# daemon-219/ReID-GAN

Measured on AMD Instinct MI355X. Metric: train-step images/sec, 256×128 ReID batch, 1/2/4/8 MI355X, higher is better.
Workload: dtype f32; 1 GPU; FD-GAN G + D_id/D_pd fwd/bwd step (FDGANModel.optimize_parameters), batch 16 pairs = 32 crops of 256x128 + 18-ch pose map per GPU, stage 2, drop 0.2; crops_per_gpu=32, global_batch_crops=32, parallelism=dp1

## Files before the change

### include/reidgan_hip.h

```cpp
#ifndef REIDGAN_HIP_H
#define REIDGAN_HIP_H

#include <stddef.h>
#include <stdint.h>

#ifdef __cplusplus
extern "C" {
#endif

typedef struct ihipStream_t* rg_stream_t;

#define RG_OK 0
#define RG_ERR_INVALID (-1)
#define RG_ERR_LAUNCH (-2)
#define RG_ERR_WORKSPACE (-3)

#define RG_ACT_NONE 0
#define RG_ACT_RELU 1
#define RG_ACT_LEAKY 2
#define RG_ACT_TANH 3

const char* rg_last_error(void);
int rg_version(void);

// ... 7 lines not shown
int rg_conv2d_fwd(const float* x, const float* w, const float* w_krsc, float* y, int N, int C, int H, int W, int K,
                  int KH, int KW, int SH, int SW, int PH, int PW, int P, int Q, const float* scale, const float* shift,
                  const float* residual, int act, float slope, void* workspace, size_t workspace_bytes,
                  rg_stream_t stream);
size_t rg_conv2d_dgrad_workspace(int N, int C, int H, int W, int K, int KH, int KW, int SH, int SW);
int rg_conv2d_dgrad(const float* dy, const float* w, const float* w_krsc, float* dx, int N, int C, int H, int W, int K,
                    int KH, int KW, int SH, int SW, int PH, int PW, int P, int Q, const float* scale,
                    const float* shift, const float* residual, int act, float slope, const float* relu_mask,
                    float* rowsum, int rowsum_cols, void* workspace, size_t workspace_bytes, rg_stream_t stream);
int rg_conv2d_dgrad_rowsum_cols(int N, int C, int H, int W, int K, int KH, int KW, int SH, int SW, int PH, int PW, int P,
                                int Q);
int rg_weights_to_krsc(const float* w, float* w_krsc, int K, int C, int KH, int KW, rg_stream_t stream);
int rg_krsc_chunk(void);
int rg_weights_to_krsc_multi(const void* table, int count, int total_blocks, rg_stream_t stream);
int rg_conv_set_force(int tile, int splits);
int rg_conv_set_planes(int mask);
int rg_conv_tune_stats(int* out);
int rg_conv_set_pick(int kind, int index);
int rg_conv_pick_log(int* buf, int max_records);
int rg_conv_splitk_arrivals(void* counters, int count, rg_stream_t stream);
int rg_conv_splitk_inkernel_count(void);
size_t rg_conv2d_wgrad_workspace(int N, int C, int K, int KH, int KW, int P, int Q);
int rg_conv2d_wgrad(const float* x, const float* dy, float* dw, int N, int C, int H, int W, int K, int KH, int KW,
                    int SH, int SW, int PH, int PW, int P, int Q, void* workspace, size_t workspace_bytes,
                    rg_stream_t stream);

size_t rg_bn_workspace(int N, int C, int HW);
int rg_bn_stats(const float* x, float* mean, float* invstd, float* running_mean, float* running_var, int N, int C,
                int HW, float eps, float momentum, void* workspace, size_t workspace_bytes, rg_stream_t stream);
int rg_bn_apply_fwd(const float* x, const float* mean, const float* stat, const float* gamma, const float* beta,
// ... 243 lines not shown
```

### reid-gan_amd/csrc/conv_igemm.hip

```cpp
#include "conv_plan.h"

#include <stdio.h>
#include <string.h>
#include <atomic>
#include <map>
#include <mutex>
#include <vector>

namespace rg {
namespace conv {

const Switches& switches() {
    static const Switches s = {
        env_int("RG_CONV_TUNE", 1),     env_int("RG_CONV_TUNE_PLAN", 1), env_int("RG_CONV_TUNE_PATH", 1), env_int("RG_CONV_TUNE8", 1),
        env_int("RG_CONV_HALO", 1),     env_int("RG_HALO_WG", 512),
        env_int("RG_THIN_CONV", 1),     env_int("RG_THIN_PX4", 1),       env_int("RG_SMALLC_PX", 1),      env_int("RG_CONV_DMA", 1),
        env_int("RG_SPLITK_VEC", 1),    env_int("RG_DGRAD_STRIDED_SPLIT", 1),
        env_int("RG_WGRAD_WG", 1024),   env_int("RG_WGRAD_XCD", 1),      env_int("RG_WGRAD_RSC", 0),      env_int("RG_WGRAD_SHIFT", 1),
        env_int("RG_WGRAD_FOLD_FUSED", 1), getenv("RG_WGRAD_WG") != nullptr,
    };
    return s;
}

static bool fits_buffer(int64_t elems) { return elems > 0 && elems * 4 < (1ll << 31); }

int validate(const char* op, const ConvGeom& g) {
    const int N = g.N, C = g.C, H = g.H, W = g.W, K = g.K, KH = g.KH, KW = g.KW, SH = g.SH, SW = g.SW, PH = g.PH, PW = g.PW, P = g.P, Q = g.Q;
    RG_REQUIRE(N > 0 && C > 0 && H > 0 && W > 0 && K > 0 && KH > 0 && KW > 0, "%s: non-positive dimension", op);
    RG_REQUIRE(SH > 0 && SW > 0 && PH >= 0 && PW >= 0 && P > 0 && Q > 0, "%s: bad stride/pad/output size", op);
    RG_REQUIRE((P - 1) * SH - PH + KH - 1 >= 0 && (Q - 1) * SW - PW + KW - 1 >= 0, "%s: inconsistent geometry", op);
    RG_REQUIRE((int64_t)(P - 1) * SH - PH < H && (int64_t)(Q - 1) * SW - PW < W, "%s: output larger than input allows", op);
    RG_REQUIRE((int64_t)N * P * Q < (1ll << 31) && (int64_t)C * KH * KW < (1ll << 31) && (int64_t)N * H * W < (1ll << 31) &&
                   (int64_t)C * H * W < (1ll << 31) && (int64_t)K * P * Q < (1ll << 31) &&
                   (int64_t)K * KH * KW < (1ll << 31),
// ... 92 lines not shown
        }
    return n;
}
size_t plans_workspace(const Plan* pl, int n, int M, int64_t Ng) {
    size_t need = 0;
    for (int i = 0; i < n; ++i) {
        const size_t b = splitk_bytes(pl[i].splits, M, Ng);
        if (b > need) need = b;
    }
    return need;
}

static Plan plan_wgrad(int M, int Ng, int64_t Kg) {
    Plan pl;
    pl.tile = (M <= 32) ? 3 : ((M <= 64 || Ng <= 64) ? 2 : 0);
    pl.m_tiles = rg::cdiv(M, kTileBM[pl.tile]);
    pl.n_tiles = rg::cdiv(Ng, kTileBN[pl.tile]);
    const int64_t nk = rg::cdiv64(Kg, BK);
    const int64_t mn = (int64_t)pl.m_tiles * pl.n_tiles;
    int64_t want = rg::cdiv64(switches().wgrad_wg, mn);
    if (want > nk / 16) want = nk / 16;
    if (want < 1) want = 1;
    if (want > 512) want = 512;
    while (want > 1 && want * (int64_t)M * Ng * 4 >= (1ll << 31)) --want;
    if (switches().wgrad_xcd && want >= 8) {
        int64_t w8 = (want + 4) / 8 * 8;
        while (w8 > 8 && w8 * (int64_t)M * Ng * 4 >= (1ll << 31)) w8 -= 8;
        if (w8 * (int64_t)M * Ng * 4 < (1ll << 31) && w8 <= nk) {
            pl.ktiles_per_split = (int)rg::cdiv64(nk, w8);
            pl.splits = (int)w8;
            return pl;
        }
    }
    pl.ktiles_per_split = (int)rg::cdiv64(nk, want);
    pl.splits = (int)rg::cdiv64(nk, pl.ktiles_per_split);
    return pl;
}

int wgrad_plan_candidates(int M, int Ng, int64_t Kg, Plan* out, int max_out) {
    out[0] = plan_wgrad(M, Ng, Kg);
    int n = 1;
    if (!plan_tune_enabled() || switches().wgrad_wg_set) return n;
    if (2.0 * M * (double)Ng * (double)Kg < kPlanTuneMinFlop) return n;
    const int64_t nk = rg::cdiv64(Kg, BK);
    const int base = out[0].splits;
    const int alts[4] = {base / 2, base * 3 / 4, base * 3 / 2, base * 2};
    for (int i = 0; i < 4 && n < max_out; ++i) {
        int64_t sp = alts[i];
        if (sp >= 8) sp = (sp + 4) / 8 * 8;
        if (sp < 1) sp = 1;
        if (sp > 512) sp = 512;
        if (sp > 1 && nk / sp < 8) continue;
        if (sp * (int64_t)M * Ng * 4 >= (1ll << 31)) continue;
        Plan pl = out[0];
        pl.ktiles_per_split = (int)rg::cdiv64(nk, sp);
        pl.splits = sp >= 8 ? (int)sp : (int)rg::cdiv64(nk, pl.ktiles_per_split);
        if (pl.splits > nk) continue;
        bool dup = false;
        for (int j = 0; j < n; ++j) dup = dup || out[j].splits == pl.splits;
        if (!dup) out[n++] = pl;
    }
    return n;
}

struct Arrivals { unsigned* ptr; int count; };
static std::map<hipStream_t, Arrivals> g_arrivals;
static std::mutex g_arrivals_mu;
static std::atomic<int> g_inkernel_launches{0};
unsigned* splitk_arrivals(hipStream_t stream, int tiles) {
    Arrivals a = {nullptr, 0};
    {
        std::lock_guard<std::mutex> lock(g_arrivals_mu);
        auto it = g_arrivals.find(stream);
        if (it != g_arrivals.end()) a = it->second;
    }
    if (!a.ptr || tiles > a.count) return nullptr;
    hipStreamCaptureStatus cs = hipStreamCaptureStatusNone;
    if (hipStreamIsCapturing(stream, &cs) != hipSuccess || cs != hipStreamCaptureStatusNone) {
        (void)hipGetLastError();
// ... 119 lines not shown
    pick_record(key, ncand, c);
    return c;
}

}
}

using namespace rg::conv;

extern "C" int rg_conv_set_force(int tile, int splits) {
    g_force_tile = tile;
    g_force_splits = splits;
    return RG_OK;
}

extern "C" int rg_conv_set_planes(int mask) {
    const int old = planes_mask();
    planes_mask() = mask & 15;
    return old;
}

extern "C" int rg_conv_set_pick(int kind, int index) {
    const int slot = pick_slot(kind);
    if (slot < 0 || index < -1) {
        rg::set_error("rg_conv_set_pick: kind %d / index %d (kinds 1, 2, 4, 16, 32, 64, 128, 256; index >= -1)", kind, index);
        return RG_ERR_INVALID - 1;
    }
    std::lock_guard<std::mutex> lock(g_pick_mu);
    const int old = g_pick[slot].exchange(index);
    if ((old >= 0) != (index >= 0)) g_pick_pinned += index >= 0 ? 1 : -1;
// ... 32 lines not shown
```

### reid-gan_amd/csrc/conv_plan.h

```cpp
#pragma once
#include "rg_common.h"

#include <array>

namespace rg {
namespace conv {

constexpr int BK = 16;
constexpr int kTileBM[4] = {128, 64, 64, 32};
constexpr int kTileBN[4] = {128, 128, 64, 256};
constexpr int kMaxCand = 16;

struct ConvGeom {
    int N, C, H, W, K, KH, KW, SH, SW, PH, PW, P, Q;
};
inline double alg_bytes(const ConvGeom& g) {
    return 4.0 * ((double)g.N * g.C * g.H * g.W + (double)g.K * g.C * g.KH * g.KW + (double)g.N * g.K * g.P * g.Q);
}
int validate(const char* op, const ConvGeom& g);

struct Workspace {
    void* ptr;
    size_t bytes;
    bool holds(size_t need) const { return need <= bytes && (!need || ptr); }
};

template <typename... P>
inline bool aligned16(const P*... p) {
    return ((... | reinterpret_cast<uintptr_t>(p)) & 15) == 0;
}

struct Switches {
    int tune, tune_plan, tune_path, tune8;
    int halo, halo_wg;
    int thin, thin_px4, smallc_px, dma;
    int splitk_vec, strided_split;
    int wgrad_wg, wgrad_xcd, wgrad_rsc, wgrad_shift, fold_fused;
    bool wgrad_wg_set;
};
const Switches& switches();
inline bool path_tune_enabled() { return switches().tune && switches().tune_path; }

struct Plan {
    int tile, m_tiles, n_tiles, splits, ktiles_per_split;
};
inline size_t splitk_bytes(int splits, int M, int64_t Ng) { return splits > 1 ? (size_t)splits * M * (size_t)Ng * sizeof(float) : 0; }
inline size_t fit_splits(Plan& pl, int M, int64_t Ng, const Workspace& ws, size_t limit = ~(size_t)0) {
    const size_t need = splitk_bytes(pl.splits, M, Ng);
    if (need < limit && ws.holds(need)) return need;
    pl.splits = 1;
    pl.ktiles_per_split = 1 << 30;
    return 0;
}
Plan plan_gemm(int M, int64_t Ng, int64_t Kg, bool allow_split);
int plan_candidates(int M, int64_t Ng, int64_t Kg, Plan* out, int max_out);
int wgrad_plan_candidates(int M, int Ng, int64_t Kg, Plan* out, int max_out);
size_t plans_workspace(const Plan* pl, int n, int M, int64_t Ng);

typedef std::array<int, 16> TuneKey;
inline TuneKey tune_key(int kind, const ConvGeom& g, int f12, int f13, int f14, int f15) {
    return TuneKey{kind, g.N, g.C, g.H, g.W, g.K, g.KH, g.KW, g.SH, g.SW, g.PH, g.PW, f12, f13, f14, f15};
}

int choose_impl(int family_bit, const TuneKey& key, hipStream_t stream, int ncand, void (*run)(void*, int), void* ctx);
template <typename Run>
inline int choose_impl(int family_bit, const TuneKey& key, hipStream_t stream, int ncand, Run run) {
    return choose_impl(family_bit, key, stream, ncand, [](void* ctx, int c) { (*static_cast<Run*>(ctx))(c); }, &run);
}
template <typename Run>
inline int choose_status(const TuneKey& key, hipStream_t stream, int ncand, Run run) {
    if (ncand <= 1) return run(0);
    int st = RG_OK;
// ... 12 lines not shown
```

### reid-gan_amd/csrc/conv_planes.h

```cpp
#pragma once
#include "conv_planes_core.h"

#ifdef RG_PLANES_FWD
template <int BM, int BN, int WM, int WN, int BMODE, bool AVEC>
__global__ __launch_bounds__(64 * WM * WN) void conv_fwd_pl_kernel(const ConvP p) {
    using T = Tile<BM, BN, WM, WN>;
    constexpr int NTH = 64 * WM * WN;
    static_assert(BN >= 64, "the gather loader needs a wave-uniform k");
    using LA = PlTile<PL_R, BM>;
    using LB = PlTile<BMODE == 2 ? PL_T : PL_R, BN>;
    constexpr int TILEB = LA::BYTES + LB::BYTES;
    __shared__ __attribute__((aligned(16))) unsigned char lds[2 * TILEB];
    const unsigned lds0 = (unsigned)(size_t)((lds_u8_t*)lds);

    const int tid = threadIdx.x, lane = tid & 63, wid = tid >> 6;
    const int wm = wid / WN, wn = wid % WN;
    const int tile = xcd_remap(blockIdx.x, gridDim.x);
    const int mt = tile % p.m_tiles, nt = tile / p.m_tiles;
    const int m0 = mt * BM, n0 = nt * BN;
    const int split = blockIdx.y;
    const int HW = p.H * p.W;
    const int RS = p.KH * p.KW;
    const rsrc_t rw = make_rsrc(p.w, p.w_bytes), rx = make_rsrc(p.x, p.x_bytes);

// ... 359 lines not shown
        ob[j] = OOB;
        if (nn < cl.Ngc) {
            const int im = fdiv(nn, cl.d_hw);
            const int rem = nn - im * cl.Hc * cl.Wc;
            const int hc = fdiv(rem, cl.d_w);
            const int wc = rem - hc * cl.Wc;
            const int h = ah + p.SH * hc, w = aw + p.SW * wc;
            ob[j] = (unsigned)((((int64_t)im * p.C + mrow0) * HW + h * p.W + w) * 4);
        }
    }
    store_tile_epilogue_any<T>(p, acc, ob, (unsigned)HW * 4u, mrow0, (cl.poff + nt) * WN + wn);
}
#endif

#ifdef RG_PLANES_WGRAD
template <int BM, int BN, int WM, int WN, bool VEC, bool VECA>
__global__ __launch_bounds__(64 * WM * WN) void conv_wgrad_pl_kernel(const ConvP p) {
    using T = Tile<BM, BN, WM, WN>;
    constexpr int NTH = 64 * WM * WN;
    static_assert(BN >= 64, "the gather loader needs a wave-uniform pixel chunk");
    using LA = PlTile<PL_R, BM>;
    using LB = PlTile<PL_R, BN>;
    constexpr int TILEB = LA::BYTES + LB::BYTES;
    __shared__ __attribute__((aligned(16))) unsigned char lds[2 * TILEB];
    const unsigned lds0 = (unsigned)(size_t)((lds_u8_t*)lds);

    const int tid = threadIdx.x, lane = tid & 63, wid = tid >> 6;
    const int wm = wid / WN, wn = wid % WN;
    int tile_id, split;
    if ((gridDim.z & 7) == 0) {
        const unsigned lin = blockIdx.z * gridDim.x + blockIdx.x;
        const unsigned xcd = lin & 7, idx = lin >> 3;
        split = (int)(xcd + 8 * (idx / gridDim.x));
        tile_id = (int)(idx % gridDim.x);
    } else {
        split = blockIdx.z;
        tile_id = xcd_remap(blockIdx.x, gridDim.x);
    }
    const int mt = tile_id % p.m_tiles, nt = tile_id / p.m_tiles;
    const int m0 = mt * BM, n0 = nt * BN;
    const rsrc_t rdy = make_rsrc(p.w, p.w_bytes), rx = make_rsrc(p.x, p.x_bytes);
    const int PQ = p.P * p.Q, HW = p.H * p.W, RS = p.KH * p.KW;
    const bool rsc = p.a_vec4 != 0;
    const bool nopad = p.PH == 0 && p.PW == 0 && (p.P - 1) * p.SH + p.KH <= p.H && (p.Q - 1) * p.SW + p.KW <= p.W;

    constexpr int AVN = (BM * 4 + NTH - 1) / NTH;
    constexpr bool AFULL = BM * 4 >= NTH;
    constexpr int EA = BM * BK / NTH;
    static_assert(VECA || EA >= 2, "scalar chunk of at least one pair");
    PlStager<VECA ? AVN : 1, VECA ? 2 : EA / 2> sa;
    const int vrow = tid >> 2, vkq = (tid & 3) * 4;
    const bool aact = AFULL || vrow < BM;
    unsigned avoff[VECA ? AVN : 1];
// ... 116 lines not shown
                const int h0 = pp * p.SH - p.PH, w0 = qq * p.SW - p.PW;
                const int xb = img * p.C * HW + h0 * p.W + w0;
                const bool ok = gvalid && cvalid && (nopad || ((unsigned)(h0 + cr) < (unsigned)p.H && (unsigned)(w0 + cs) < (unsigned)p.W));
                rb[e] = bload(rx, ok ? (unsigned)(xb + coff) * 4u : OOB);
                if (++qq == p.Q) {
                    qq = 0;
                    if (++pp == p.P) { pp = 0; ++img; }
                }
            }
        }
    };

    constexpr int SA = decltype(sa)::STEPS, S = SA + decltype(sb)::STEPS;
    const unsigned fa = lds0 + LA::frag_base(lane, wm * T::WTM), fb = lds0 + LA::BYTES + LB::frag_base(lane, wn * T::WTN);
    const int nk_total = (p.Kg + BK - 1) / BK;
    const int kt_begin = split * p.ktiles_per_split;
    int kt_end = kt_begin + p.ktiles_per_split;
    if (kt_end > nk_total) kt_end = nk_total;
    pl_mainloop<T, LA, LB, S>(fa, fb, kt_begin, kt_end, acc, load_tile, [&](unsigned wbuf, int s) {
        if (s < SA) {
            if constexpr (AFULL || !VECA) sa.step(s, ra, wbuf, LA::PIECE);
            else sa.step(s, ra, wbuf, LA::PIECE, aact);
        } else {
            sb.step(s - SA, rb, wbuf, LB::PIECE);
        }
    });

    const int l32 = lane & 31, kh = lane >> 5;
    const rsrc_t ro = make_rsrc(p.y, p.y_bytes);
    const int mrow0 = m0 + wm * T::WTM + 4 * kh;
    const unsigned rstride = (unsigned)p.Ng * 4u;
#pragma unroll
    for (int j = 0; j < T::TN; ++j) {
        const int nn = n0 + wn * T::WTN + j * 32 + l32;
        const unsigned ob = nn < p.Ng ? (unsigned)((((int64_t)split * p.M + mrow0) * p.Ng + nn) * 4) : OOB;
#pragma unroll
        for (int i = 0; i < T::TM; ++i)
#pragma unroll
            for (int r = 0; r < 16; ++r) {
                const int mo = i * 32 + (r & 3) + 8 * (r >> 2);
                bstore(ro, (mrow0 + mo < p.M) ? ob + (unsigned)mo * rstride : OOB, acc[i][j][r]);
            }
    }
}
#endif
```

### reid-gan_amd/csrc/conv_planes_core.h

```cpp
#pragma once

enum { PL_R = 0, PL_T = 1 };

typedef int int2r __attribute__((ext_vector_type(2)));
typedef short short4r __attribute__((ext_vector_type(4)));
typedef __attribute__((address_space(3))) short4r lds_short4_t;
typedef __attribute__((address_space(3))) int4r lds_int4_t;
typedef __attribute__((address_space(3))) int2r lds_int2_t;
typedef __attribute__((address_space(3))) int lds_int_t;
typedef __attribute__((address_space(3))) unsigned char lds_u8_t;
template <bool B> struct BoolTag { static constexpr bool value = B; };

constexpr int pl_tpitch(int rows) {
    const int p = rows * 2, b = p / 256 * 256;
    return b + 64 >= p ? b + 64 : (b + 192 >= p ? b + 192 : b + 320);
}

template <int KIND, int ROWS>
struct PlTile {
    static constexpr int HALF = ROWS * 16 + 64;
    static constexpr int PITCH = pl_tpitch(ROWS);
    static constexpr int PIECE = KIND == PL_R ? 2 * HALF : 16 * PITCH;
    static constexpr int BYTES = 3 * PIECE;
    static constexpr int BLK = KIND == PL_R ? 512 : 64;
// ... 292 lines not shown
    __syncthreads();
    pl_kloop(kt_begin, kt_end, load_tile, [&](auto cur_tag, auto stage_tag) {
        constexpr int RD = decltype(cur_tag)::value ? TILEB : 0, WR = TILEB - RD;
        constexpr bool STAGE = decltype(stage_tag)::value;
        mma_pl16<T::TM, T::TN>([&](int i, int pc) { return LA::frag(fa[i & 1] + RD + pc * LA::PIECE + (i >> 1) * 2 * LA::BLK); },
                               [&](int j, int pc) { return LB::frag(fb[j & 1] + RD + pc * LB::PIECE + (j >> 1) * 2 * LB::BLK); }, acc,
                               [&](int slot) {
                                   if (STAGE) {
#pragma unroll
                                       for (int s = pl_first_step<S, NM>(slot); s < pl_end_step<S, NM>(slot); ++s)
                                           if (s >= 0) stage(WR, s);
                                   }
                               });
    });
}
```

### reid-gan_amd/csrc/conv_wgrad.hip

```cpp
#define RG_PLANES_WGRAD
#include "conv_thin.h"

namespace {

template <int KH, int KW, int KO>
__global__ __launch_bounds__(256) void conv_wgrad_k1_kernel(const ThinP t) {
    constexpr int RS = KH * KW;
    __shared__ float red[4][KO * RS];
    const int Ng = t.N * t.P * t.Q;
    const int PQ = t.P * t.Q;
    const int c = blockIdx.x;
    const int beg = blockIdx.y * t.per_slice;
    const int end = min(beg + t.per_slice, Ng);
    const rsrc_t rx = make_rsrc(t.x, t.x_bytes);
    float acc[KO][KH][KW];
#pragma unroll
    for (int k = 0; k < KO; ++k)
#pragma unroll
        for (int r = 0; r < KH; ++r)
#pragma unroll
            for (int s = 0; s < KW; ++s) acc[k][r][s] = 0.f;
    for (int pix = beg + threadIdx.x; pix < end; pix += 256) {
        const int img = fdiv(pix, t.d_pq);
        const int pq = pix - img * PQ;
// ... 438 lines not shown
        reinterpret_cast<float4*>(out)[i] = v;
        return;
    }
    const int64_t crs = (int64_t)C * RS;
    const float vv[4] = {v.x, v.y, v.z, v.w};
#pragma unroll
    for (int j = 0; j < 4; ++j) {
        const int64_t e = i * 4 + j;
        const int64_t m = e / crs;
        const int np = (int)(e - m * crs);
        const int rs = np / C, c = np - rs * C;
        out[m * crs + (int64_t)c * RS + rs] = vv[j];
    }
}

__global__ __launch_bounds__(256) void splitk_reduce_fold_kernel(const float* __restrict__ ws, float* __restrict__ out,
                                                                 const float* __restrict__ w, int M, int64_t n, int splits,
                                                                 const float* __restrict__ scale, const float* __restrict__ invstd,
                                                                 const float* __restrict__ mean, const float* __restrict__ sum_g,
                                                                 const float* __restrict__ part, int S, float* __restrict__ dbeta,
                                                                 float* __restrict__ dgamma) {
    __shared__ float4 red[4][64];
    __shared__ float redf[16];
    const int k = blockIdx.x;
    const int tx = threadIdx.x & 63, ty = threadIdx.x >> 6;
    const int M4 = M >> 2;
    const int64_t n4 = n >> 2;
    const float4* w4 = reinterpret_cast<const float4*>(ws);
    const float4* f4 = reinterpret_cast<const float4*>(w);
    float4* o4 = reinterpret_cast<float4*>(out);
    const float sc = scale[k];
    float dot = 0.f;
    for (int c0 = 0; c0 < M4; c0 += 64) {
        const int c = c0 + tx;
        const int64_t i = (int64_t)k * M4 + c;
        float4 s0 = make_float4(0.f, 0.f, 0.f, 0.f), s1 = s0;
        if (c < M4) {
            int q = ty;
            for (; q + 12 < splits; q += 16) {
                const float4 a = w4[(int64_t)q * n4 + i], b = w4[(int64_t)(q + 4) * n4 + i];
                const float4 cc = w4[(int64_t)(q + 8) * n4 + i], d = w4[(int64_t)(q + 12) * n4 + i];
                s0.x += a.x; s0.y += a.y; s0.z += a.z; s0.w += a.w;
                s1.x += b.x; s1.y += b.y; s1.z += b.z; s1.w += b.w;
                s0.x += cc.x; s0.y += cc.y; s0.z += cc.z; s0.w += cc.w;
                s1.x += d.x; s1.y += d.y; s1.z += d.z; s1.w += d.w;
            }
            for (; q + 4 < splits; q += 8) {
                const float4 a = w4[(int64_t)q * n4 + i], b = w4[(int64_t)(q + 4) * n4 + i];
                s0.x += a.x; s0.y += a.y; s0.z += a.z; s0.w += a.w;
                s1.x += b.x; s1.y += b.y; s1.z += b.z; s1.w += b.w;
            }
            if (q < splits) {
                const float4 a = w4[(int64_t)q * n4 + i];
                s0.x += a.x; s0.y += a.y; s0.z += a.z; s0.w += a.w;
            }
        }
        red[ty][tx] = make_float4(s0.x + s1.x, s0.y + s1.y, s0.z + s1.z, s0.w + s1.w);
        __syncthreads();
        if (ty == 0 && c < M4) {
            const float4 r0 = red[0][tx], r1 = red[1][tx], r2 = red[2][tx], r3 = red[3][tx];
            const float4 v = make_float4((r0.x + r1.x) + (r2.x + r3.x), (r0.y + r1.y) + (r2.y + r3.y), (r0.z + r1.z) + (r2.z + r3.z),
                                         (r0.w + r1.w) + (r2.w + r3.w));
            if (dgamma) {
                const float4 wv = f4[i];
                dot += (wv.x * v.x + wv.y * v.y) + (wv.z * v.z + wv.w * v.w);
            }
            o4[i] = make_float4(v.x * sc, v.y * sc, v.z * sc, v.w * sc);
        }
        __syncthreads();
    }
    float sg = 0.f;
    if (part) {
        float t = 0.f;
        for (int s = threadIdx.x; s < S; s += 256) t += part[(int64_t)k * S + s];
        sg = rg_block_sum(t, redf);
        if (dbeta && threadIdx.x == 0) dbeta[k] = sg;
    } else if (sum_g) {
        sg = sum_g[k];
    }
    if (dgamma) {
        const float t = rg_block_sum(dot, redf);
        if (threadIdx.x == 0) dgamma[k] = invstd[k] * (t - mean[k] * sg);
    }
}

#include "conv_planes.h"

}

using namespace rg::conv;

extern "C" int rg_weights_to_krsc(const float* w, float* w_krsc, int K, int C, int KH, int KW, hipStream_t stream) {
    RG_REQUIRE(w && w_krsc && K > 0 && C > 0 && KH > 0 && KW > 0, "rg_weights_to_krsc: bad arguments");
    const int64_t total = (int64_t)K * C * KH * KW;
    rg::ProfScope prof(rg::FAM_MISC, stream, 0.0, 8.0 * total);
    hipLaunchKernelGGL(weights_to_krsc_kernel, dim3(finish_grid(total)), dim3(256), 0, stream, w, w_krsc, total, C,
                       KH * KW);
// ... 7 lines not shown
    rg::ProfScope prof(rg::FAM_CONV_FWD, stream, 0.0, 8.0 * (double)total_blocks * KRSC_CHUNK);
    hipLaunchKernelGGL(weights_to_krsc_multi_kernel, dim3(total_blocks), dim3(256), 0, stream, static_cast<const long long*>(table),
                       count);
    return rg::check_launch("rg_weights_to_krsc_multi");
}

extern "C" int rg_bn_fold_wgrad(const float* w, float* g, const float* scale, const float* invstd, const float* running_mean,
                                const float* sum_g, const float* partials, int n_slices, float* dbeta, float* dgamma, int K,
                                int M, hipStream_t stream);

#define RG_WGRAD_LAUNCH_K(KERNEL, NTH, BM_, BN_, WM_, WN_)                                                          \
    if (vec) hipLaunchKernelGGL((KERNEL<BM_, BN_, WM_, WN_, true, true>), grid, dim3(NTH), 0, stream, p);           \
    else if (veca) hipLaunchKernelGGL((KERNEL<BM_, BN_, WM_, WN_, false, true>), grid, dim3(NTH), 0, stream, p);    \
    else hipLaunchKernelGGL((KERNEL<BM_, BN_, WM_, WN_, false, false>), grid, dim3(NTH), 0, stream, p)
#define RG_WGRAD_LAUNCH(BM_, BN_, WM_, WN_) RG_WGRAD_LAUNCH_K(conv_wgrad_kernel, NT, BM_, BN_, WM_, WN_)
#define RG_WGRAD_PL_LAUNCH(BM_, BN_, WM_, WN_) RG_WGRAD_LAUNCH_K(conv_wgrad_pl_kernel, 64 * WM_ * WN_, BM_, BN_, WM_, WN_)
#define RG_WGRAD_TILE_SWITCH(tile, LAUNCH)     \
    switch (tile) {                            \
        case 0: LAUNCH(128, 128, 2, 2); break; \
        case 2: LAUNCH(64, 64, 2, 2); break;   \
        default: LAUNCH(32, 256, 1, 4); break; \
    }

namespace {

static bool thin_px4(const ConvGeom& g, const float* dy) {
    return switches().thin_px4 && g.KH == 3 && g.KW == 3 && g.SH == 1 && g.SW == 1 && g.PH <= 1 && g.PW <= 1 && (g.Q & 3) == 0 &&
           g.Q + 2 - 2 * g.PW == g.W && aligned16(dy) && ((g.P * g.Q) & 3) == 0;
}
#define THIN_PX4_DISPATCH(KERNEL, g, grid, stream, t)                                                 \
    do {                                                                                              \
        if (g.K == 1) hipLaunchKernelGGL((KERNEL<1>), grid, dim3(256), 0, stream, t);                 \
        else if (g.K == 2) hipLaunchKernelGGL((KERNEL<2>), grid, dim3(256), 0, stream, t);            \
        else if (g.K == 3) hipLaunchKernelGGL((KERNEL<3>), grid, dim3(256), 0, stream, t);            \
        else hipLaunchKernelGGL((KERNEL<4>), grid, dim3(256), 0, stream, t);                          \
    } while (0)
static int thin_wgrad_per_slice(int C, int64_t Ng) {
    int64_t slices = rg::cdiv64(2048, C);
    if (slices > Ng / 512) slices = Ng / 512;
    if (slices < 1) slices = 1;
    return (int)((rg::cdiv64(Ng, slices) + 3) / 4 * 4);
}

static void launch_reduce(hipStream_t stream, const float* ws, float* out, int64_t n, int splits, int rsc, int C, int RS) {
    if (switches().splitk_vec && aligned16(ws, out) && (n & 3) == 0)
        hipLaunchKernelGGL(splitk_reduce_vec_kernel, dim3((unsigned)rg::cdiv64(n >> 2, 64)), dim3(256), 0, stream, ws, out, n, splits, rsc,
                           C, RS);
    else
        hipLaunchKernelGGL(splitk_reduce_kernel, dim3((unsigned)rg::cdiv64(n, 64)), dim3(256), 0, stream, ws, out, n, splits, rsc, C, RS);
}

struct FoldArgs {
    const float *w, *scale, *invstd, *mean, *sum_g, *partials;
    int n_slices;
    float *dbeta, *dgamma;
};
// ... 27 lines not shown
    else THIN_DISPATCH(conv_wgrad_k1_kernel, g, grid, c.stream, t);
    if (int e = rg::check_launch("rg_conv2d_wgrad(thin)")) return e;
    launch_reduce(c.stream, static_cast<const float*>(c.ws.ptr), c.o.dw, (int64_t)g.K * c.p.Ng, slices, 0, g.C, g.KH * g.KW);
    if (int e = rg::check_launch("rg_conv2d_wgrad(thin reduce)")) return e;
    return fold ? fold_after(fold, c.o.dw, g.K, c.p.Ng, c.stream) : RG_OK;
}

static int wgrad_run_plan(const WgradCall& c, const Plan& pl) {
    const ConvGeom& g = c.g;
    const FoldArgs* fold = c.o.fold;
    hipStream_t stream = c.stream;
    float* dw = c.o.dw;
    ConvP p = c.p;
    p.m_tiles = pl.m_tiles; p.n_tiles = pl.n_tiles;
    p.splits = pl.splits; p.ktiles_per_split = pl.ktiles_per_split;
    const size_t need = (size_t)pl.splits * p.M * (size_t)p.Ng * sizeof(float);
    if (need > c.ws.bytes || !c.ws.ptr) {
        rg::set_error("rg_conv2d_wgrad: workspace too small (%zu < %zu)", c.ws.bytes, need);
        return RG_ERR_WORKSPACE;
    }
    RG_REQUIRE(need < (1ull << 31), "rg_conv2d_wgrad: partial buffer exceeds 2 GiB");
    const bool rsc = switches().wgrad_rsc && (g.KH * g.KW > 1) && (g.C % 16 == 0);
    const bool via_ws = pl.splits > 1 || rsc;
    float* const partial = static_cast<float*>(c.ws.ptr);
    p.a_vec4 = rsc ? 1 : 0;
    p.y = via_ws ? partial : dw;
    p.x_bytes = x_bytes(g);
    p.w_bytes = y_bytes(g);
    p.y_bytes = via_ws ? (unsigned)need : w_bytes(g);
    const dim3 grid(p.m_tiles * p.n_tiles, 1, pl.splits);
    {
        rg::ProfScope prof(rg::FAM_CONV_WGRAD, stream, 2.0 * p.M * (double)p.Ng * p.Kg, alg_bytes(g));
        const bool veca = aligned16(c.o.x, c.o.dy) && ((g.P * g.Q) % 4 == 0);
        bool vec = veca && g.KH == 1 && g.KW == 1 && g.SH == 1 && g.SW == 1 && g.PH == 0 && g.PW == 0;
        if (!vec && !rsc && switches().wgrad_shift && veca && g.SH == 1 && g.SW == 1 && g.PW <= 1 && g.KW <= g.PW + 2 && g.Q % 4 == 0 &&
            g.W >= 4 && g.KW * g.KH > 1) {
            vec = true;
            p.wshift = 1;
        }
        const TuneKey tk = tune_key(4, g, (vec ? 2 : 0) + (veca ? 1 : 0) + p.wshift * 4, pl.tile, pl.splits, 0);
        choose_impl(4, tk, stream, pl.tile == 0 ? 3 : 2, [&](int impl) {
            if (impl == 2) { RG_WGRAD_PL_LAUNCH(128, 128, 4, 2); }
            else if (impl) { RG_WGRAD_TILE_SWITCH(pl.tile, RG_WGRAD_PL_LAUNCH); }
            else { RG_WGRAD_TILE_SWITCH(pl.tile, RG_WGRAD_LAUNCH); }
        });
        if (int e = rg::check_launch("rg_conv2d_wgrad")) return e;
        if (via_ws) {
            const int64_t n = (int64_t)p.M * p.Ng;
            if (fold && !rsc && (p.Ng & 3) == 0 && aligned16(partial, dw, fold->w) && switches().fold_fused) {
                hipLaunchKernelGGL(splitk_reduce_fold_kernel, dim3(p.M), dim3(256), 0, stream, partial, dw, fold->w, p.Ng, n, pl.splits,
                                   fold->scale, fold->invstd, fold->mean, fold->sum_g, fold->partials, fold->n_slices, fold->dbeta,
                                   fold->dgamma);
                return rg::check_launch("rg_conv2d_wgrad(reduce + fold)");
            }
            launch_reduce(stream, partial, dw, n, pl.splits, rsc ? 1 : 0, g.C, g.KH * g.KW);
        }
    }
    if (int e = rg::check_launch("rg_conv2d_wgrad(reduce)")) return e;
    return fold ? fold_after(fold, dw, g.K, g.C * g.KH * g.KW, stream) : RG_OK;
}

int wgrad_impl(const ConvGeom& g, const WgradOps& o, const Workspace& ws, hipStream_t stream) {
    if (int e = validate("rg_conv2d_wgrad", g)) return e;
    RG_REQUIRE(o.x && o.dy && o.dw, "rg_conv2d_wgrad: null tensor");
    RG_REQUIRE(g.KH < 65536 && g.KW < 65536, "rg_conv2d_wgrad: filter too large");
    WgradCall c = {g, o, ws, stream};
    ConvP& p = c.p;
    fill_common(p, g);
    p.x = o.x; p.w = o.dy;
    p.ep = Epilogue{nullptr, nullptr, nullptr, 0, 0.f, nullptr, nullptr, 0};
// ... 47 lines not shown
```

Baseline: 936.9 images/s.

## Add in-workgroup k-group split for wgrad and rework reduce-fold kernel

The planes wgrad kernel can now run 2 or 4 k-groups per workgroup. Each group handles its own k-range, and the accumulators are summed through LDS before a single slab is written, which cuts the split-K partial buffer and the reduce traffic. The fused split-K reduce+fold kernel moves to 512 threads and can pack several output rows per block for small Ng. A force override for wgrad tile/splits and an API to set kgroups are added. Trade-offs are higher LDS and thread counts per workgroup, extra barriers, and lower occupancy.

```diff
diff --git a/include/reidgan_hip.h b/include/reidgan_hip.h
--- a/include/reidgan_hip.h
+++ b/include/reidgan_hip.h
@@ -45,6 +45,7 @@
 int rg_krsc_chunk(void);
 int rg_weights_to_krsc_multi(const void* table, int count, int total_blocks, rg_stream_t stream);
 int rg_conv_set_force(int tile, int splits);
+int rg_conv_set_wgrad_kgroups(int kgroups, int fold_fused);
 int rg_conv_set_planes(int mask);
 int rg_conv_tune_stats(int* out);
 int rg_conv_set_pick(int kind, int index);
diff --git a/reid-gan_amd/csrc/conv_igemm.hip b/reid-gan_amd/csrc/conv_igemm.hip
--- a/reid-gan_amd/csrc/conv_igemm.hip
+++ b/reid-gan_amd/csrc/conv_igemm.hip
@@ -17,7 +17,7 @@
         env_int("RG_THIN_CONV", 1),     env_int("RG_THIN_PX4", 1),       env_int("RG_SMALLC_PX", 1),      env_int("RG_CONV_DMA", 1),
         env_int("RG_SPLITK_VEC", 1),    env_int("RG_DGRAD_STRIDED_SPLIT", 1),
         env_int("RG_WGRAD_WG", 1024),   env_int("RG_WGRAD_XCD", 1),      env_int("RG_WGRAD_RSC", 0),      env_int("RG_WGRAD_SHIFT", 1),
-        env_int("RG_WGRAD_FOLD_FUSED", 1), getenv("RG_WGRAD_WG") != nullptr,
+        env_int("RG_WGRAD_FOLD_FUSED", 1), env_int("RG_WGRAD_KGROUPS", 0), getenv("RG_WGRAD_WG") != nullptr,
     };
     return s;
 }
@@ -140,6 +140,9 @@
 static Plan plan_wgrad(int M, int Ng, int64_t Kg) {
     Plan pl;
     pl.tile = (M <= 32) ? 3 : ((M <= 64 || Ng <= 64) ? 2 : 0);
+    int ftile = -1, fsplits = -1;
+    force_override(&ftile, &fsplits);
+    if (ftile == 0 || ftile == 2 || ftile == 3) pl.tile = ftile;
     pl.m_tiles = rg::cdiv(M, kTileBM[pl.tile]);
     pl.n_tiles = rg::cdiv(Ng, kTileBN[pl.tile]);
     const int64_t nk = rg::cdiv64(Kg, BK);
@@ -149,6 +152,13 @@
     if (want < 1) want = 1;
     if (want > 512) want = 512;
     while (want > 1 && want * (int64_t)M * Ng * 4 >= (1ll << 31)) --want;
+    if (fsplits >= 1) {
+        want = fsplits < nk ? fsplits : nk;
+        while (want > 1 && want * (int64_t)M * Ng * 4 >= (1ll << 31)) --want;
+        pl.ktiles_per_split = (int)rg::cdiv64(nk, want);
+        pl.splits = (int)rg::cdiv64(nk, pl.ktiles_per_split);
+        return pl;
+    }
     if (switches().wgrad_xcd && want >= 8) {
         int64_t w8 = (want + 4) / 8 * 8;
         while (w8 > 8 && w8 * (int64_t)M * Ng * 4 >= (1ll << 31)) w8 -= 8;
@@ -166,7 +176,7 @@
 int wgrad_plan_candidates(int M, int Ng, int64_t Kg, Plan* out, int max_out) {
     out[0] = plan_wgrad(M, Ng, Kg);
     int n = 1;
-    if (!plan_tune_enabled() || switches().wgrad_wg_set) return n;
+    if (g_force_tile >= 0 || g_force_splits >= 1 || !plan_tune_enabled() || switches().wgrad_wg_set) return n;
     if (2.0 * M * (double)Ng * (double)Kg < kPlanTuneMinFlop) return n;
     const int64_t nk = rg::cdiv64(Kg, BK);
     const int base = out[0].splits;
@@ -189,6 +199,16 @@
     return n;
 }
 
+static std::atomic<int> g_wgrad_kgroups{-1}, g_wgrad_fold_fused{-1};
+int wgrad_kgroups_forced() {
+    const int v = g_wgrad_kgroups.load();
+    return v >= 0 ? v : switches().wgrad_kgroups;
+}
+bool wgrad_fold_fused() {
+    const int v = g_wgrad_fold_fused.load();
+    return v >= 0 ? v != 0 : switches().fold_fused != 0;
+}
+
 struct Arrivals { unsigned* ptr; int count; };
 static std::map<hipStream_t, Arrivals> g_arrivals;
 static std::mutex g_arrivals_mu;
@@ -338,6 +358,14 @@
     return RG_OK;
 }
 
+extern "C" int rg_conv_set_wgrad_kgroups(int kgroups, int fold_fused) {
+    RG_REQUIRE(kgroups == -1 || kgroups == 0 || kgroups == 1 || kgroups == 2 || kgroups == 4, "rg_conv_set_wgrad_kgroups: kgroups must be -1, 0, 1, 2 or 4");
+    RG_REQUIRE(fold_fused >= -1 && fold_fused <= 1, "rg_conv_set_wgrad_kgroups: fold_fused must be -1, 0 or 1");
+    g_wgrad_kgroups = kgroups;
+    g_wgrad_fold_fused = fold_fused;
+    return RG_OK;
+}
+
 extern "C" int rg_conv_set_planes(int mask) {
     const int old = planes_mask();
     planes_mask() = mask & 15;
diff --git a/reid-gan_amd/csrc/conv_plan.h b/reid-gan_amd/csrc/conv_plan.h
--- a/reid-gan_amd/csrc/conv_plan.h
+++ b/reid-gan_amd/csrc/conv_plan.h
@@ -36,6 +36,7 @@
     int thin, thin_px4, smallc_px, dma;
     int splitk_vec, strided_split;
     int wgrad_wg, wgrad_xcd, wgrad_rsc, wgrad_shift, fold_fused;
+    int wgrad_kgroups;
     bool wgrad_wg_set;
 };
 const Switches& switches();
@@ -56,6 +57,8 @@
 int plan_candidates(int M, int64_t Ng, int64_t Kg, Plan* out, int max_out);
 int wgrad_plan_candidates(int M, int Ng, int64_t Kg, Plan* out, int max_out);
 size_t plans_workspace(const Plan* pl, int n, int M, int64_t Ng);
+int wgrad_kgroups_forced();
+bool wgrad_fold_fused();
 
 typedef std::array<int, 16> TuneKey;
 inline TuneKey tune_key(int kind, const ConvGeom& g, int f12, int f13, int f14, int f15) {
diff --git a/reid-gan_amd/csrc/conv_planes.h b/reid-gan_amd/csrc/conv_planes.h
--- a/reid-gan_amd/csrc/conv_planes.h
+++ b/reid-gan_amd/csrc/conv_planes.h
@@ -397,29 +397,36 @@
 #endif
 
 #ifdef RG_PLANES_WGRAD
-template <int BM, int BN, int WM, int WN, bool VEC, bool VECA>
-__global__ __launch_bounds__(64 * WM * WN) void conv_wgrad_pl_kernel(const ConvP p) {
+template <int BM, int BN, int WM, int WN, bool VEC, bool VECA, int KG = 1>
+__global__ __launch_bounds__(64 * WM * WN * KG) void conv_wgrad_pl_kernel(const ConvP p) {
     using T = Tile<BM, BN, WM, WN>;
     constexpr int NTH = 64 * WM * WN;
     static_assert(BN >= 64, "the gather loader needs a wave-uniform pixel chunk");
+    static_assert(KG == 1 || KG == 2 || KG == 4, "1, 2 or 4 k-groups");
+    static_assert(NTH * KG <= 1024, "at most 16 waves per workgroup");
     using LA = PlTile<PL_R, BM>;
     using LB = PlTile<PL_R, BN>;
     constexpr int TILEB = LA::BYTES + LB::BYTES;
-    __shared__ __attribute__((aligned(16))) unsigned char lds[2 * TILEB];
-    const unsigned lds0 = (unsigned)(size_t)((lds_u8_t*)lds);
-
-    const int tid = threadIdx.x, lane = tid & 63, wid = tid >> 6;
+    static_assert(KG * 2 * TILEB <= 160 * 1024, "operand tiles of all k-groups in 160 KiB of LDS");
+    static_assert((KG - 1) * BM * BN * 4 <= KG * 2 * TILEB, "the accumulator hand-over fits the operand buffers");
+    __shared__ __attribute__((aligned(16))) unsigned char lds[KG * 2 * TILEB];
+    const unsigned ldsb = (unsigned)(size_t)((lds_u8_t*)lds);
+    const int grp = KG == 1 ? 0 : __builtin_amdgcn_readfirstlane((int)threadIdx.x / NTH);
+    const unsigned lds0 = ldsb + (unsigned)grp * (2u * TILEB);
+
+    const int tid = KG == 1 ? (int)threadIdx.x : (int)threadIdx.x - grp * NTH, lane = tid & 63, wid = tid >> 6;
     const int wm = wid / WN, wn = wid % WN;
-    int tile_id, split;
+    int tile_id, slab;
     if ((gridDim.z & 7) == 0) {
         const unsigned lin = blockIdx.z * gridDim.x + blockIdx.x;
         const unsigned xcd = lin & 7, idx = lin >> 3;
-        split = (int)(xcd + 8 * (idx / gridDim.x));
+        slab = (int)(xcd + 8 * (idx / gridDim.x));
         tile_id = (int)(idx % gridDim.x);
     } else {
-        split = blockIdx.z;
+        slab = blockIdx.z;
         tile_id = xcd_remap(blockIdx.x, gridDim.x);
     }
+    const int split = slab * KG + grp;
     const int mt = tile_id % p.m_tiles, nt = tile_id / p.m_tiles;
     const int m0 = mt * BM, n0 = nt * BN;
     const rsrc_t rdy = make_rsrc(p.w, p.w_bytes), rx = make_rsrc(p.x, p.x_bytes);
@@ -566,7 +573,8 @@
     constexpr int SA = decltype(sa)::STEPS, S = SA + decltype(sb)::STEPS;
     const unsigned fa = lds0 + LA::frag_base(lane, wm * T::WTM), fb = lds0 + LA::BYTES + LB::frag_base(lane, wn * T::WTN);
     const int nk_total = (p.Kg + BK - 1) / BK;
-    const int kt_begin = split * p.ktiles_per_split;
+    int kt_begin = split * p.ktiles_per_split;
+    if (KG > 1 && (split >= p.splits || kt_begin > nk_total)) kt_begin = nk_total;
     int kt_end = kt_begin + p.ktiles_per_split;
     if (kt_end > nk_total) kt_end = nk_total;
     pl_mainloop<T, LA, LB, S>(fa, fb, kt_begin, kt_end, acc, load_tile, [&](unsigned wbuf, int s) {
@@ -577,6 +585,12 @@
             sb.step(s - SA, rb, wbuf, LB::PIECE);
         }
     });
+    if constexpr (KG > 1) {
+        const int n0 = min(p.ktiles_per_split, nk_total - slab * KG * p.ktiles_per_split), n = kt_end - kt_begin;
+        for (int i = (n > 1 ? n : 1); i < (n0 > 1 ? n0 : 1); ++i) __syncthreads();
+        pl_kgroup_sum<T, KG, NTH>(ldsb, grp, tid, acc);
+        if (grp != 0) return;
+    }
 
     const int l32 = lane & 31, kh = lane >> 5;
     const rsrc_t ro = make_rsrc(p.y, p.y_bytes);
@@ -585,7 +599,7 @@
 #pragma unroll
     for (int j = 0; j < T::TN; ++j) {
         const int nn = n0 + wn * T::WTN + j * 32 + l32;
-        const unsigned ob = nn < p.Ng ? (unsigned)((((int64_t)split * p.M + mrow0) * p.Ng + nn) * 4) : OOB;
+        const unsigned ob = nn < p.Ng ? (unsigned)((((int64_t)slab * p.M + mrow0) * p.Ng + nn) * 4) : OOB;
 #pragma unroll
         for (int i = 0; i < T::TM; ++i)
 #pragma unroll
diff --git a/reid-gan_amd/csrc/conv_planes_core.h b/reid-gan_amd/csrc/conv_planes_core.h
--- a/reid-gan_amd/csrc/conv_planes_core.h
+++ b/reid-gan_amd/csrc/conv_planes_core.h
@@ -330,3 +330,40 @@
                                });
     });
 }
+
+typedef __attribute__((address_space(3))) floatx4 lds_f4_t;
+template <typename T, int KG, int NTH>
+__device__ __forceinline__ void pl_kgroup_sum(unsigned base, int grp, int tid, floatx16 (&acc)[T::TM][T::TN]) {
+    constexpr int NQ = T::TM * T::TN * 4;
+    constexpr unsigned GROUPB = (unsigned)NTH * NQ * 16u;
+    __syncthreads();
+    if (grp != 0) {
+        const unsigned a = base + (unsigned)(grp - 1) * GROUPB + (unsigned)tid * 16u;
+#pragma unroll
+        for (int i = 0; i < T::TM; ++i)
+#pragma unroll
+            for (int j = 0; j < T::TN; ++j)
+#pragma unroll
+                for (int q = 0; q < 4; ++q) {
+                    const floatx16& c = acc[i][j];
+                    *(lds_f4_t*)(size_t)(a + (unsigned)(((i * T::TN + j) * 4 + q) * NTH) * 16u) =
+                        floatx4{c[4 * q], c[4 * q + 1], c[4 * q + 2], c[4 * q + 3]};
+                }
+    }
+    __syncthreads();
+    if (grp != 0) return;
+#pragma unroll
+    for (int g = 1; g < KG; ++g) {
+        const unsigned a = base + (unsigned)(g - 1) * GROUPB + (unsigned)tid * 16u;
+#pragma unroll
+        for (int i = 0; i < T::TM; ++i)
+#pragma unroll
+            for (int j = 0; j < T::TN; ++j)
+#pragma unroll
+                for (int q = 0; q < 4; ++q) {
+                    const floatx4 v = *(const lds_f4_t*)(size_t)(a + (unsigned)(((i * T::TN + j) * 4 + q) * NTH) * 16u);
+                    floatx16& c = acc[i][j];
+                    c[4 * q] += v[0]; c[4 * q + 1] += v[1]; c[4 * q + 2] += v[2]; c[4 * q + 3] += v[3];
+                }
+    }
+}
diff --git a/reid-gan_amd/csrc/conv_wgrad.hip b/reid-gan_amd/csrc/conv_wgrad.hip
--- a/reid-gan_amd/csrc/conv_wgrad.hip
+++ b/reid-gan_amd/csrc/conv_wgrad.hip
@@ -476,73 +476,98 @@
     }
 }
 
-__global__ __launch_bounds__(256) void splitk_reduce_fold_kernel(const float* __restrict__ ws, float* __restrict__ out,
-                                                                 const float* __restrict__ w, int M, int64_t n, int splits,
-                                                                 const float* __restrict__ scale, const float* __restrict__ invstd,
-                                                                 const float* __restrict__ mean, const float* __restrict__ sum_g,
-                                                                 const float* __restrict__ part, int S, float* __restrict__ dbeta,
-                                                                 float* __restrict__ dgamma) {
-    __shared__ float4 red[4][64];
-    __shared__ float redf[16];
-    const int k = blockIdx.x;
-    const int tx = threadIdx.x & 63, ty = threadIdx.x >> 6;
+__global__ __launch_bounds__(512) void splitk_reduce_fold_kernel(const float* __restrict__ ws, float* __restrict__ out,
+                                                                 const float* __restrict__ w, int K, int M, int64_t n, int splits,
+                                                                 int segshift, const float* __restrict__ scale,
+                                                                 const float* __restrict__ invstd, const float* __restrict__ mean,
+                                                                 const float* __restrict__ sum_g, const float* __restrict__ part, int S,
+                                                                 float* __restrict__ dbeta, float* __restrict__ dgamma) {
+    __shared__ float4 red[2][8][64];
+    __shared__ float sgs[64];
+    const int tx = threadIdx.x & 63, ch = threadIdx.x >> 6;
     const int M4 = M >> 2;
     const int64_t n4 = n >> 2;
+    const int seg = 1 << segshift, R = 64 >> segshift;
+    const int k = blockIdx.x * R + (tx >> segshift), col = tx & (seg - 1);
+    const bool rowok = k < K;
+    const int nch = R > 1 ? 1 : (M4 + 63) >> 6;
     const float4* w4 = reinterpret_cast<const float4*>(ws);
     const float4* f4 = reinterpret_cast<const float4*>(w);
     float4* o4 = reinterpret_cast<float4*>(out);
-    const float sc = scale[k];
+    const float sc = (ch == 0 && rowok) ? scale[k] : 0.f;
     float dot = 0.f;
-    for (int c0 = 0; c0 < M4; c0 += 64) {
-        const int c = c0 + tx;
+    for (int it = 0; it < nch; ++it) {
+        const int c = it * 64 + col;
+        const bool ok = rowok && c < M4;
         const int64_t i = (int64_t)k * M4 + c;
-        float4 s0 = make_float4(0.f, 0.f, 0.f, 0.f), s1 = s0;
-        if (c < M4) {
-            int q = ty;
-            for (; q + 12 < splits; q += 16) {
-                const float4 a = w4[(int64_t)q * n4 + i], b = w4[(int64_t)(q + 4) * n4 + i];
-                const float4 cc = w4[(int64_t)(q + 8) * n4 + i], d = w4[(int64_t)(q + 12) * n4 + i];
-                s0.x += a.x; s0.y += a.y; s0.z += a.z; s0.w += a.w;
-                s1.x += b.x; s1.y += b.y; s1.z += b.z; s1.w += b.w;
-                s0.x += cc.x; s0.y += cc.y; s0.z += cc.z; s0.w += cc.w;
-                s1.x += d.x; s1.y += d.y; s1.z += d.z; s1.w += d.w;
-            }
-            for (; q + 4 < splits; q += 8) {
-                const float4 a = w4[(int64_t)q * n4 + i], b = w4[(int64_t)(q + 4) * n4 + i];
-                s0.x += a.x; s0.y += a.y; s0.z += a.z; s0.w += a.w;
-                s1.x += b.x; s1.y += b.y; s1.z += b.z; s1.w += b.w;
-            }
-            if (q < splits) {
-                const float4 a = w4[(int64_t)q * n4 + i];
-                s0.x += a.x; s0.y += a.y; s0.z += a.z; s0.w += a.w;
-            }
-        }
-        red[ty][tx] = make_float4(s0.x + s1.x, s0.y + s1.y, s0.z + s1.z, s0.w + s1.w);
+        float4 s = make_float4(0.f, 0.f, 0.f, 0.f);
+        if (ok) {
+            const float4* src = w4 + i;
+            int q = ch;
+            for (; q + 56 < splits; q += 64) {
+                float4 a[8];
+#pragma unroll
+                for (int u = 0; u < 8; ++u) a[u] = src[(int64_t)(q + 8 * u) * n4];
+#pragma unroll
+                for (int u = 0; u < 8; ++u) { s.x += a[u].x; s.y += a[u].y; s.z += a[u].z; s.w += a[u].w; }
+            }
+            if (q + 24 < splits) {
+                float4 a[4];
+#pragma unroll
+                for (int u = 0; u < 4; ++u) a[u] = src[(int64_t)(q + 8 * u) * n4];
+#pragma unroll
+                for (int u = 0; u < 4; ++u) { s.x += a[u].x; s.y += a[u].y; s.z += a[u].z; s.w += a[u].w; }
+                q += 32;
+            }
+            for (; q < splits; q += 8) {
+                const float4 a = src[(int64_t)q * n4];
+                s.x += a.x; s.y += a.y; s.z += a.z; s.w += a.w;
+            }
+        }
+        red[it & 1][ch][tx] = s;
         __syncthreads();
-        if (ty == 0 && c < M4) {
-            const float4 r0 = red[0][tx], r1 = red[1][tx], r2 = red[2][tx], r3 = red[3][tx];
-            const float4 v = make_float4((r0.x + r1.x) + (r2.x + r3.x), (r0.y + r1.y) + (r2.y + r3.y), (r0.z + r1.z) + (r2.z + r3.z),
-                                         (r0.w + r1.w) + (r2.w + r3.w));
+        if (ch == 0 && ok) {
+            float4 r[4];
+#pragma unroll
+            for (int t = 0; t < 4; ++t) {
+                const float4 a = red[it & 1][t][tx], b = red[it & 1][t + 4][tx];
+                r[t] = make_float4(a.x + b.x, a.y + b.y, a.z + b.z, a.w + b.w);
+            }
+            const float4 v = make_float4((r[0].x + r[1].x) + (r[2].x + r[3].x), (r[0].y + r[1].y) + (r[2].y + r[3].y),
+                                         (r[0].z + r[1].z) + (r[2].z + r[3].z), (r[0].w + r[1].w) + (r[2].w + r[3].w));
             if (dgamma) {
                 const float4 wv = f4[i];
                 dot += (wv.x * v.x + wv.y * v.y) + (wv.z * v.z + wv.w * v.w);
             }
             o4[i] = make_float4(v.x * sc, v.y * sc, v.z * sc, v.w * sc);
         }
-        __syncthreads();
-    }
-    float sg = 0.f;
-    if (part) {
-        float t = 0.f;
-        for (int s = threadIdx.x; s < S; s += 256) t += part[(int64_t)k * S + s];
-        sg = rg_block_sum(t, redf);
-        if (dbeta && threadIdx.x == 0) dbeta[k] = sg;
-    } else if (sum_g) {
-        sg = sum_g[k];
-    }
-    if (dgamma) {
-        const float t = rg_block_sum(dot, redf);
-        if (threadIdx.x == 0) dgamma[k] = invstd[k] * (t - mean[k] * sg);
+    }
+    for (int r = ch; r < R; r += 8) {
+        const int kr = blockIdx.x * R + r;
+        if (kr >= K) break;
+        float sg = 0.f;
+        if (part) {
+            for (int v = 0; v < 4; ++v) {
+                float t = 0.f;
+                for (int s = v * 64 + tx; s < S; s += 256) t += part[(int64_t)kr * S + s];
+                sg += rg_wave_sum(t);
+            }
+            if (dbeta && tx == 0) dbeta[kr] = sg;
+        } else if (sum_g) {
+            sg = sum_g[kr];
+        }
+        if (tx == 0) sgs[r] = sg;
+    }
+    __syncthreads();
+    if (dgamma && ch == 0) {
+        float t = dot;
+#pragma unroll
+        for (int off = 32; off > 0; off >>= 1) {
+            const float o = __shfl_xor(t, off, 64);
+            t += off < seg ? o : 0.f;
+        }
+        t = 0.f + t;
+        if (rowok && col == 0) dgamma[k] = invstd[k] * (t - mean[k] * sgs[tx >> segshift]);
     }
 }
 
@@ -580,7 +605,13 @@
     else if (veca) hipLaunchKernelGGL((KERNEL<BM_, BN_, WM_, WN_, false, true>), grid, dim3(NTH), 0, stream, p);    \
     else hipLaunchKernelGGL((KERNEL<BM_, BN_, WM_, WN_, false, false>), grid, dim3(NTH), 0, stream, p)
 #define RG_WGRAD_LAUNCH(BM_, BN_, WM_, WN_) RG_WGRAD_LAUNCH_K(conv_wgrad_kernel, NT, BM_, BN_, WM_, WN_)
-#define RG_WGRAD_PL_LAUNCH(BM_, BN_, WM_, WN_) RG_WGRAD_LAUNCH_K(conv_wgrad_pl_kernel, 64 * WM_ * WN_, BM_, BN_, WM_, WN_)
+#define RG_WGRAD_PL_LAUNCH_G(BM_, BN_, WM_, WN_, KG_)                                                                                   \
+    if (vec) hipLaunchKernelGGL((conv_wgrad_pl_kernel<BM_, BN_, WM_, WN_, true, true, KG_>), grid, dim3(64 * WM_ * WN_ * KG_), 0, stream, p);           \
+    else if (veca) hipLaunchKernelGGL((conv_wgrad_pl_kernel<BM_, BN_, WM_, WN_, false, true, KG_>), grid, dim3(64 * WM_ * WN_ * KG_), 0, stream, p);    \
+    else hipLaunchKernelGGL((conv_wgrad_pl_kernel<BM_, BN_, WM_, WN_, false, false, KG_>), grid, dim3(64 * WM_ * WN_ * KG_), 0, stream, p)
+#define RG_WGRAD_PL_LAUNCH_G2(BM_, BN_, WM_, WN_)                                  \
+    if (kg == 2) { RG_WGRAD_PL_LAUNCH_G(BM_, BN_, WM_, WN_, 2); }                  \
+    else { RG_WGRAD_PL_LAUNCH_G(BM_, BN_, WM_, WN_, 1); }
 #define RG_WGRAD_TILE_SWITCH(tile, LAUNCH)     \
     switch (tile) {                            \
         case 0: LAUNCH(128, 128, 2, 2); break; \
@@ -606,6 +637,17 @@
     if (slices > Ng / 512) slices = Ng / 512;
     if (slices < 1) slices = 1;
     return (int)((rg::cdiv64(Ng, slices) + 3) / 4 * 4);
+}
+
+static int wgrad_kgroups(int impl, const Plan& pl) {
+    if (impl == 0 || pl.splits < 2) return 1;
+    const int forced = wgrad_kgroups_forced();
+    if (forced > 0) {
+        int g = (impl == 1 && pl.tile == 2) ? 4 : 2;
+        while (g > forced || g > pl.splits) g >>= 1;
+        return g;
+    }
+    return ((pl.splits & 7) == 0 && ((pl.splits / 2) & 7) != 0) ? 1 : 2;
 }
 
 static void launch_reduce(hipStream_t stream, const float* ws, float* out, int64_t n, int splits, int rsc, int C, int RS) {
@@ -663,21 +705,22 @@
     ConvP p = c.p;
     p.m_tiles = pl.m_tiles; p.n_tiles = pl.n_tiles;
     p.splits = pl.splits; p.ktiles_per_split = pl.ktiles_per_split;
-    const size_t need = (size_t)pl.splits * p.M * (size_t)p.Ng * sizeof(float);
-    if (need > c.ws.bytes || !c.ws.ptr) {
+    const bool rsc = switches().wgrad_rsc && (g.KH * g.KW > 1) && (g.C % 16 == 0);
+    const auto slabs_of = [&](int impl) { return rg::cdiv(pl.splits, wgrad_kgroups(impl, pl)); };
+    int max_slabs = 1;
+    for (int impl = 0; impl < (pl.tile == 0 ? 3 : 2); ++impl) max_slabs = slabs_of(impl) > max_slabs ? slabs_of(impl) : max_slabs;
+    const size_t need = (size_t)max_slabs * p.M * (size_t)p.Ng * sizeof(float);
+    const bool any_ws = max_slabs > 1 || rsc;
+    if (any_ws && (need > c.ws.bytes || !c.ws.ptr)) {
         rg::set_error("rg_conv2d_wgrad: workspace too small (%zu < %zu)", c.ws.bytes, need);
         return RG_ERR_WORKSPACE;
     }
     RG_REQUIRE(need < (1ull << 31), "rg_conv2d_wgrad: partial buffer exceeds 2 GiB");
-    const bool rsc = switches().wgrad_rsc && (g.KH * g.KW > 1) && (g.C % 16 == 0);
-    const bool via_ws = pl.splits > 1 || rsc;
     float* const partial = static_cast<float*>(c.ws.ptr);
     p.a_vec4 = rsc ? 1 : 0;
-    p.y = via_ws ? partial : dw;
     p.x_bytes = x_bytes(g);
     p.w_bytes = y_bytes(g);
-    p.y_bytes = via_ws ? (unsigned)need : w_bytes(g);
-    const dim3 grid(p.m_tiles * p.n_tiles, 1, pl.splits);
+    const int tiles = p.m_tiles * p.n_tiles;
     {
         rg::ProfScope prof(rg::FAM_CONV_WGRAD, stream, 2.0 * p.M * (double)p.Ng * p.Kg, alg_bytes(g));
         const bool veca = aligned16(c.o.x, c.o.dy) && ((g.P * g.Q) % 4 == 0);
@@ -688,21 +731,39 @@
             p.wshift = 1;
         }
         const TuneKey tk = tune_key(4, g, (vec ? 2 : 0) + (veca ? 1 : 0) + p.wshift * 4, pl.tile, pl.splits, 0);
-        choose_impl(4, tk, stream, pl.tile == 0 ? 3 : 2, [&](int impl) {
-            if (impl == 2) { RG_WGRAD_PL_LAUNCH(128, 128, 4, 2); }
-            else if (impl) { RG_WGRAD_TILE_SWITCH(pl.tile, RG_WGRAD_PL_LAUNCH); }
+        const int ran = choose_impl(4, tk, stream, pl.tile == 0 ? 3 : 2, [&](int impl) {
+            const int kg = wgrad_kgroups(impl, pl), slabs = rg::cdiv(pl.splits, kg);
+            const bool to_ws = slabs > 1 || rsc;
+            p.y = to_ws ? partial : dw;
+            p.y_bytes = to_ws ? (unsigned)((size_t)slabs * p.M * (size_t)p.Ng * sizeof(float)) : w_bytes(g);
+            const dim3 grid(tiles, 1, slabs);
+            if (impl == 2) { RG_WGRAD_PL_LAUNCH_G2(128, 128, 4, 2); }
+            else if (impl) {
+                switch (pl.tile) {
+                    case 0: RG_WGRAD_PL_LAUNCH_G2(128, 128, 2, 2); break;
+                    case 2:
+                        if (kg == 4) { RG_WGRAD_PL_LAUNCH_G(64, 64, 2, 2, 4); }
+                        else { RG_WGRAD_PL_LAUNCH_G2(64, 64, 2, 2); }
+                        break;
+                    default: RG_WGRAD_PL_LAUNCH_G2(32, 256, 1, 4); break;
+                }
+            }
             else { RG_WGRAD_TILE_SWITCH(pl.tile, RG_WGRAD_LAUNCH); }
         });
         if (int e = rg::check_launch("rg_conv2d_wgrad")) return e;
-        if (via_ws) {
+        const int slabs = slabs_of(ran);
+        if (slabs > 1 || rsc) {
             const int64_t n = (int64_t)p.M * p.Ng;
-            if (fold && !rsc && (p.Ng & 3) == 0 && aligned16(partial, dw, fold->w) && switches().fold_fused) {
-                hipLaunchKernelGGL(splitk_reduce_fold_kernel, dim3(p.M), dim3(256), 0, stream, partial, dw, fold->w, p.Ng, n, pl.splits,
-                                   fold->scale, fold->invstd, fold->mean, fold->sum_g, fold->partials, fold->n_slices, fold->dbeta,
-                                   fold->dgamma);
+            if (fold && !rsc && (p.Ng & 3) == 0 && aligned16(partial, dw, fold->w) && wgrad_fold_fused()) {
+                const int M4 = p.Ng >> 2;
+                int segshift = 6;
+                if (M4 <= 32) for (segshift = 0; (1 << segshift) < M4; ++segshift) {}
+                hipLaunchKernelGGL(splitk_reduce_fold_kernel, dim3(rg::cdiv(p.M, 64 >> segshift)), dim3(512), 0, stream, partial, dw,
+                                   fold->w, p.M, p.Ng, n, slabs, segshift, fold->scale, fold->invstd, fold->mean, fold->sum_g,
+                                   fold->partials, fold->n_slices, fold->dbeta, fold->dgamma);
                 return rg::check_launch("rg_conv2d_wgrad(reduce + fold)");
             }
-            launch_reduce(stream, partial, dw, n, pl.splits, rsc ? 1 : 0, g.C, g.KH * g.KW);
+            launch_reduce(stream, partial, dw, n, slabs, rsc ? 1 : 0, g.C, g.KH * g.KW);
         }
     }
     if (int e = rg::check_launch("rg_conv2d_wgrad(reduce)")) return e;
```

Measured after the change: 888.5 images/s. 0.948x the previous value.
